# Jeremy-Cleland/hmer-img2latex

Hardware: AMD Instinct MI355X
Metric: decoded LaTeX tokens/sec at batch 256, 320x64 imgs, seq 150 (higher is better)
Workload: dtype f32

## Files before the change

### hmer-img2latex_amd/csrc/api.hip

```cpp
#include "common.h"
#include <new>

extern "C" int i2l_version(void) { return 110; }

extern "C" const char* i2l_error_string(int code) {
    switch (code) {
        case I2L_OK: return "ok";
        case I2L_ERR_ARG: return "invalid argument (null pointer or non-positive dimension)";
        case I2L_ERR_UNSUPPORTED: return "dimension not supported by the gfx950 kernels";
        case I2L_ERR_WORKSPACE: return "workspace missing or too small";
        case I2L_ERR_LAUNCH: return "HIP launch error";
        default: return "unknown error";
    }
}

struct i2l_lanes {
    int n = 0;
    hipStream_t s[I2L_MAX_LANES] = {};
    hipEvent_t fork[I2L_MAX_LANES] = {}, join[I2L_MAX_LANES] = {};
};

extern "C" int i2l_lanes_create(const i2l_stream_t* streams, int n, i2l_lanes** out) {
    if (!streams || !out || n < 1 || n > I2L_MAX_LANES) return I2L_ERR_ARG;
    for (int i = 0; i < n; ++i)
        if (!streams[i]) return I2L_ERR_ARG;
    i2l_lanes* l = new (std::nothrow) i2l_lanes();
    if (!l) return I2L_ERR_WORKSPACE;
    l->n = n;
    bool ok = true;
    for (int i = 0; i < n; ++i) {
        l->s[i] = i2l_s(streams[i]);
        ok = ok && hipEventCreateWithFlags(&l->fork[i], hipEventDisableTiming) == hipSuccess;
        ok = ok && hipEventCreateWithFlags(&l->join[i], hipEventDisableTiming) == hipSuccess;
    }
    if (!ok) { i2l_lanes_destroy(l); return I2L_ERR_LAUNCH; }
    *out = l;
// ... 48 lines not shown
```

### hmer-img2latex_amd/csrc/common.h

```cpp
#pragma once
#include <hip/hip_runtime.h>
#include <stdint.h>

#include "../../include/img2latex_hip.h"

#define I2L_CHECK_LAUNCH()                                   \
    do {                                                     \
        if (hipGetLastError() != hipSuccess) return I2L_ERR_LAUNCH; \
    } while (0)

static inline hipStream_t i2l_s(i2l_stream_t s) { return reinterpret_cast<hipStream_t>(s); }
hipStream_t i2l_side_fork(i2l_lanes* lanes, hipStream_t main, int lane);
#include <atomic>
static inline bool i2l_lds_attr(const void* fn, size_t bytes, std::atomic<unsigned>& done) {
    int dev = 0;
    if (hipGetDevice(&dev) != hipSuccess) return false;
    if (dev >= 0 && dev < 32 && ((done.load(std::memory_order_relaxed) >> dev) & 1u)) return true;
    if (hipFuncSetAttribute(fn, hipFuncAttributeMaxDynamicSharedMemorySize, (int)bytes) != hipSuccess) return false;
    if (dev >= 0 && dev < 32) done.fetch_or(1u << dev, std::memory_order_relaxed);
    return true;
}
static inline int i2l_cdiv(int a, int b) { return (a + b - 1) / b; }
static inline size_t i2l_align(size_t x, size_t a = 256) { return (x + a - 1) / a * a; }

struct GemmArgs {
    const float* A; long lda; int a_kc;
    const float* W; long ldw; int w_kc;
    long bsa, bsw; int nz;
    const float* bias;
    const float* bias2;
    float* C; int ldc;
    int M, N, K;
    int relu;
    int perm_h;
    float alpha;
    int accumulate;
    int split_bf16;
    int conv_h, conv_w;
    const float* pool_y;
    const unsigned char* pool_am;
    const float* scale;
    const float* residual;
};
static inline GemmArgs gemm_args() {
    GemmArgs g{};
    g.a_kc = 1; g.w_kc = 1; g.nz = 1; g.alpha = 1.f;
    return g;
}
size_t i2l_gemm_workspace_bytes(int M, int N, int K, int nz = 1);
int i2l_gemm(const GemmArgs& g, void* ws, size_t ws_bytes, hipStream_t s);
bool i2l_gemm_split_bf16_ok(const GemmArgs& g);

bool i2l_conv_bf16x3_applicable(int Cin, int Cout);
bool i2l_conv_bf16x3_full_applicable(int Cin, int Cout);
size_t i2l_conv_bf16x3_workspace_bytes(int Cin, int Cout);
int i2l_conv_bf16x3_run(const float* x, const float* w, const float* bias, float* y, unsigned char* amax, int B, int Cin,
                        int H, int W, int Cout, void* workspace, size_t workspace_bytes, hipStream_t s, int full = 0,
                        int weights_packed = 0);
bool i2l_conv_smallk_applicable(int Cin, int Cout);
int i2l_conv_smallk_run(const float* x, const float* w, const float* bias, float* y, unsigned char* amax, int B, int Cin,
                        int H, int W, int Cout, void* workspace, size_t workspace_bytes, hipStream_t s);
size_t i2l_conv_fixlist_bytes(void);
```

### hmer-img2latex_amd/csrc/decode.hip

```cpp
#include <math.h>
#include <stdlib.h>

#include "common.h"

namespace {

#include "lstm_rows.inc.h"

constexpr int MAXL = I2L_MAX_LSTM_LAYERS;
constexpr int NT = 256;
constexpr int VCHUNK = 2 * NT;

constexpr size_t GROUP_STATUS_BYTES = 2048;
inline bool group_shape_ok(int V, int H, int L) { return L == 1 && H == 256 && V <= 512; }

__global__ __launch_bounds__(256) void transpose_perm_kernel(const float* __restrict__ W, int N, int K,
                                                             float* __restrict__ out, int ld_out, int Npad,
                                                             int perm_h) {
    __shared__ float tile[64][65];
    const int c0 = blockIdx.x * 64, k0 = blockIdx.y * 64;
    const int tx = threadIdx.x & 63, ty = threadIdx.x >> 6;
    for (int i = ty; i < 64; i += 4) {
        const int c = c0 + i, k = k0 + tx;
        const int n = perm_h > 0 ? (c & 3) * perm_h + (c >> 2) : c;
// ... 717 lines not shown
        hipLaunchKernelGGL(transpose_perm_kernel, grid, dim3(256), 0, s, w->w_out, V, H, F(lo.WoutT), lo.Vp, lo.Vp, 0);
        I2L_CHECK_LAUNCH();
        hipLaunchKernelGGL(bout_pad_kernel, dim3(i2l_cdiv(lo.Vp, 256)), dim3(256), 0, s, w->b_out, F(lo.boutP), V, lo.Vp);
        I2L_CHECK_LAUNCH();
        if (lo.wpack16) {
            hipLaunchKernelGGL(pack16_kernel, dim3(16 * 4), dim3(64), 0, s, F(lo.WhhT[0]), F(lo.WoutT),
                               reinterpret_cast<u32x4_t*>(base + lo.wpack16));
            I2L_CHECK_LAUNCH();
        }
    }
    const size_t gws = lo.total - lo.gemm_ws;
    if (what & I2L_PREP_WEIGHTS) {
        GemmArgs g = gemm_args();
        g.A = w->embedding; g.lda = E;
        g.W = w->w_ih[0]; g.ldw = 2 * E;
        g.C = F(lo.P); g.ldc = G;
        g.M = V; g.N = G; g.K = E; g.perm_h = H;
        rc = i2l_gemm(g, base + lo.gemm_ws, gws, s);
        if (rc != I2L_OK) return rc;
    }
    if (what & I2L_PREP_ROWS) {
        GemmArgs g = gemm_args();
        g.A = enc; g.lda = E;
        g.W = w->w_ih[0] + E; g.ldw = 2 * E;
        g.bias = w->b_ih[0]; g.bias2 = w->b_hh[0];
        g.C = F(lo.Genc); g.ldc = G;
        g.M = rows; g.N = G; g.K = E; g.perm_h = H;
        rc = i2l_gemm(g, base + lo.gemm_ws, gws, s);
        if (rc != I2L_OK) return rc;
    }
    return I2L_OK;
}

namespace {
int launch_decode(const i2l_decoder_weights* w, const void* workspace, int rows, int steps, const int32_t* tok0,
                  const int32_t* forced, const float* h0, const float* c0, float temperature, int select, int stop,
                  int end_id, int top_k, float top_p, unsigned long long seed, int32_t* ids_out, float* logits_out,
                  float* probs_out, float* h_out, float* c_out, i2l_stream_t stream, int rows_per_wg = 0, int flags = 0,
                  uint32_t* resident_flag = nullptr, uint32_t resident_value = 0);
}

extern "C" int i2l_greedy_decode_ex(const i2l_decoder_weights* w, const void* workspace, int rows, int steps,
                                    const int32_t* tok0, const int32_t* forced, const float* h0, const float* c0,
                                    float temperature, int select, int stop, int end_id, int rows_per_workgroup,
                                    int32_t* ids_out, float* logits_out, float* h_out, float* c_out, int flags,
                                    uint32_t* resident_flag, uint32_t resident_value, i2l_stream_t stream) {
    if (select != I2L_SELECT_LOGITS && select != I2L_SELECT_SOFTMAX) return I2L_ERR_ARG;
    if (rows_per_workgroup != 0 && rows_per_workgroup != 1 && rows_per_workgroup != 2 && rows_per_workgroup != 4)
        return I2L_ERR_ARG;
    return launch_decode(w, workspace, rows, steps, tok0, forced, h0, c0, temperature, select, stop, end_id, 0, 0.f, 0ull,
                         ids_out, logits_out, nullptr, h_out, c_out, stream, rows_per_workgroup, flags, resident_flag,
                         resident_value);
}

extern "C" int i2l_greedy_decode(const i2l_decoder_weights* w, const void* workspace, int rows, int steps,
                                 const int32_t* tok0, const int32_t* forced, const float* h0, const float* c0,
                                 float temperature, int select, int stop, int end_id, int32_t* ids_out,
                                 float* logits_out, float* h_out, float* c_out, i2l_stream_t stream) {
    if (select != I2L_SELECT_LOGITS && select != I2L_SELECT_SOFTMAX) return I2L_ERR_ARG;
    return launch_decode(w, workspace, rows, steps, tok0, forced, h0, c0, temperature, select, stop, end_id, 0, 0.f, 0ull,
                         ids_out, logits_out, nullptr, h_out, c_out, stream);
}

extern "C" int i2l_sample_decode(const i2l_decoder_weights* w, const void* workspace, int rows, int steps,
                                 const int32_t* tok0, const float* h0, const float* c0, float temperature, int top_k,
                                 float top_p, uint64_t seed, int stop, int end_id, int32_t* ids_out, float* probs_out,
// ... 540 lines not shown
```

### hmer-img2latex_amd/csrc/gemm.hip

```cpp
#include <stdlib.h>

#include "common.h"

namespace {

#include "bf16_split.inc.h"

constexpr int BM = 64, BN = 64, BK = 64, LDP = BK + 1;
constexpr int NLD = BM * BK / 4 / 256;
constexpr int KQ = BK / 4;
typedef float f32x16 __attribute__((ext_vector_type(16)));

__host__ __device__ __forceinline__ size_t slab_stride(int M, int N) {
    size_t units = ((size_t)M * N + 63) / 64;
    if ((units & 1) == 0) ++units;
    return units * 64;
}

__device__ __forceinline__ int perm_col(int n, int perm_h) {
    if (perm_h <= 0) return n;
    const int g = n / perm_h, j = n - g * perm_h;
    return 4 * j + g;
}

// ... 428 lines not shown

int run_bf16x3(const GemmArgs& g, void* ws, size_t ws_bytes, hipStream_t s) {
    int S, kc;
    plan_bf16x3(g.M, g.N, (long)g.nz * g.K, &S, &kc);
    if (S > 1 && (!ws || ws_bytes < (size_t)S * slab_stride(g.M, g.N) * sizeof(float))) return I2L_ERR_WORKSPACE;
    const int mt = bf16x3_mt(g.M);
    const int tiles_n = i2l_cdiv(g.N, LBN), tiles = i2l_cdiv(g.M, 64 * mt) * tiles_n;
    const long long blocks = (long long)tiles * S;
    if (blocks > 0x7fffffffll) return I2L_ERR_UNSUPPORTED;
    dim3 grid((unsigned)blocks);
    float* wsf = static_cast<float*>(ws);
    const bool plain = g.nz == 1 && !g.pool_y && g.conv_h <= 0;
    if (!plain && (g.scale || g.residual)) return I2L_ERR_UNSUPPORTED;
#define I2L_LAUNCH_BF16X3(AK, WK)                                                                                          \
    do {                                                                                                                \
        if (mt == 2 && plain) hipLaunchKernelGGL((gemm_bf16x3_kernel<AK, WK, 2, true>), grid, dim3(256), 0, s, g, wsf, kc, S, tiles_n, tiles); \
        else if (mt == 2) hipLaunchKernelGGL((gemm_bf16x3_kernel<AK, WK, 2, false>), grid, dim3(256), 0, s, g, wsf, kc, S, tiles_n, tiles); \
        else if (plain) hipLaunchKernelGGL((gemm_bf16x3_kernel<AK, WK, 1, true>), grid, dim3(256), 0, s, g, wsf, kc, S, tiles_n, tiles); \
        else hipLaunchKernelGGL((gemm_bf16x3_kernel<AK, WK, 1, false>), grid, dim3(256), 0, s, g, wsf, kc, S, tiles_n, tiles);  \
    } while (0)
    if (g.a_kc && g.w_kc) I2L_LAUNCH_BF16X3(true, true);
    else if (g.a_kc) I2L_LAUNCH_BF16X3(true, false);
    else if (g.w_kc) I2L_LAUNCH_BF16X3(false, true);
    else I2L_LAUNCH_BF16X3(false, false);
#undef I2L_LAUNCH_BF16X3
    I2L_CHECK_LAUNCH();
    if (S > 1) {
        launch_splitk_reduce(g, (const float*)ws, S, s);
        I2L_CHECK_LAUNCH();
    }
    return I2L_OK;
}

}

bool i2l_gemm_split_bf16_ok(const GemmArgs& g0) {
    GemmArgs g = g0;
    if (g.nz < 1) g.nz = 1;
    return g.split_bf16 && bf16x3_applicable(g);
}

size_t i2l_gemm_workspace_bytes(int M, int N, int K, int nz) {
    int ks, kc;
    plan(M, N, K, nz < 1 ? 1 : nz, &ks, &kc);
    const size_t slabs = (size_t)ks * (nz < 1 ? 1 : nz);
    size_t need = slabs > 1 ? i2l_align(slabs * slab_stride(M, N) * sizeof(float)) : 0;
    if (K >= 64) {
        int S, kc;
        plan_bf16x3(M, N, (long)(nz < 1 ? 1 : nz) * K, &S, &kc);
        const size_t n3 = S > 1 ? i2l_align((size_t)S * slab_stride(M, N) * sizeof(float)) : 0;
        if (n3 > need) need = n3;
    }
    return need;
}

int i2l_gemm(const GemmArgs& g0, void* ws, size_t ws_bytes, hipStream_t stream) {
    GemmArgs g = g0;
    if (!g.A || !g.W || !g.C || g.M <= 0 || g.N <= 0 || g.K <= 0) return I2L_ERR_ARG;
    if (g.nz < 1) g.nz = 1;
    if (g.split_bf16 && bf16x3_applicable(g)) return run_bf16x3(g, ws, ws_bytes, stream);
    int ks, kc;
    plan(g.M, g.N, g.K, g.nz, &ks, &kc);
    const int slabs = ks * g.nz;
    if (slabs > 65535) return I2L_ERR_UNSUPPORTED;
    if (slabs > 1 && (!ws || ws_bytes < (size_t)slabs * slab_stride(g.M, g.N) * sizeof(float))) return I2L_ERR_WORKSPACE;
    auto al16 = [](const void* p) { return reinterpret_cast<uintptr_t>(p) % 16 == 0; };
// ... 123 lines not shown
```

### hmer-img2latex_amd/img2latex_amd/_lib.py

```python
from __future__ import annotations

import ctypes
import os
from ctypes import POINTER, c_char_p, c_double, c_float, c_int, c_int32, c_size_t, c_uint64, c_void_p
from typing import Optional, Sequence

import torch

_HERE = os.path.dirname(os.path.abspath(__file__))
LIB_PATH = os.path.join(_HERE, "libimg2latex_hip.so")

OK = 0
ERR_ARG, ERR_UNSUPPORTED, ERR_WORKSPACE, ERR_LAUNCH = -1, -2, -3, -4
STOP_NONE, STOP_STICKY = 0, 1
SELECT_LOGITS, SELECT_SOFTMAX, SELECT_SAMPLE = 0, 1, 2
PREP_WEIGHTS, PREP_ROWS, PREP_ALL = 1, 2, 3
MAX_LSTM_LAYERS, MAX_BEAM, MAX_NBEST = 4, 8, 16
FLAG_EXACT_FP32, FLAG_NO_GROUP, FLAG_RESNET_NO_RING, FLAG_RESNET_IM2COL_STEM = 0x1, 0x2, 0x4, 0x8
FLAG_WEIGHTS_PACKED = 0x10
FLAG_AGENT_SCOPE_EXCHANGE = 0x20
FLAG_CONV_NO_SPARSE_WGRAD = 0x4000
FLAG_CONV_COL_READY = 0x10000
FLAG_DECODE_REGION_CLEARED = 0x2000000
FLAG_RESNET_WIDE_TILES = 0x40000
# ... 32 lines not shown

_SIGNATURES = {
    "i2l_version": (c_int, []),
    "i2l_error_string": (c_char_p, [c_int]),
    "i2l_lanes_create": (c_int, [POINTER(c_void_p), c_int, POINTER(c_void_p)]),
    "i2l_lanes_destroy": (c_int, [c_void_p]),
    "i2l_lanes_join": (c_int, [c_void_p, c_void_p]),
    "i2l_stream_wait_value32": (c_int, [c_void_p, ctypes.c_uint32, ctypes.c_float, c_void_p]),
    "i2l_conv_workspace_bytes": (c_size_t, [c_int, c_int]),
    "i2l_conv3x3_relu_pool2_fwd": (c_int, [c_void_p, c_void_p, c_void_p, c_void_p, c_void_p, c_int, c_int, c_int,
                                           c_int, c_int, c_void_p, c_size_t, c_int, c_void_p]),
    "i2l_conv_bwd_workspace_bytes": (c_size_t, [c_int, c_int, c_int, c_int, c_int]),
    "i2l_conv3x3_relu_pool2_bwd": (c_int, [c_void_p, c_void_p, c_void_p, c_void_p, c_void_p, c_void_p, c_void_p,
                                           c_void_p, c_int, c_int, c_int, c_int, c_int, c_void_p, c_size_t, c_int,
                                           c_void_p, c_void_p]),
    "i2l_linear_bwd_workspace_bytes": (c_size_t, [c_int, c_int, c_int]),
    "i2l_linear_bias_act_bwd": (c_int, [c_void_p, c_void_p, c_void_p, c_void_p, c_void_p, c_void_p, c_void_p, c_int,
                                        c_int, c_int, c_int, c_void_p, c_size_t, c_int, c_void_p, c_void_p]),
    "i2l_linear_workspace_bytes": (c_size_t, [c_int, c_int, c_int]),
    "i2l_linear_bias_act_fwd": (c_int, [c_void_p, c_void_p, c_void_p, c_void_p, c_int, c_int, c_int, c_int,
                                        c_void_p, c_size_t, c_int, c_void_p]),
    "i2l_conv_bf16_packed_bytes": (c_size_t, [c_int] * 4),
    "i2l_conv_bn_bf16_pack": (c_int, [c_void_p, c_void_p, c_void_p, c_void_p, c_void_p, c_float, c_void_p, c_size_t,
                                      c_int, c_int, c_int, c_int, c_void_p]),
    "i2l_conv_bf16_workspace_bytes": (c_size_t, [c_int] * 10),
    "i2l_conv_bn_act_bf16_fwd": (c_int, [c_void_p, c_int, c_void_p, c_void_p, c_void_p] + [c_int] * 10 +
                                 [c_void_p, c_size_t, c_int, c_void_p]),
    "i2l_bottleneck_join_bf16_fwd": (c_int, [c_void_p, c_void_p, c_void_p, c_void_p, c_void_p, c_void_p, ctypes.c_long,
                                             c_int, c_int, c_int, c_void_p]),
    "i2l_maxpool3x3s2_bf16_fwd": (c_int, [c_void_p, c_void_p, c_int, c_int, c_int, c_int, c_void_p]),
    "i2l_global_avgpool_bf16_fwd": (c_int, [c_void_p, c_void_p, c_int, c_int, c_int, c_int, c_void_p]),
    "i2l_decoder_workspace_bytes": (c_size_t, [c_int, c_int, c_int, c_int, c_int]),
    "i2l_decoder_prepare": (c_int, [POINTER(DecoderWeights), c_void_p, c_int, c_int, c_void_p, c_size_t, c_void_p]),
    "i2l_greedy_decode": (c_int, [POINTER(DecoderWeights), c_void_p, c_int, c_int, c_void_p, c_void_p, c_void_p,
                                  c_void_p, c_float, c_int, c_int, c_int, c_void_p, c_void_p, c_void_p, c_void_p,
                                  c_void_p]),
    "i2l_greedy_decode_ex": (c_int, [POINTER(DecoderWeights), c_void_p, c_int, c_int, c_void_p, c_void_p, c_void_p,
                                     c_void_p, c_float, c_int, c_int, c_int, c_int, c_void_p, c_void_p, c_void_p,
                                     c_void_p, c_int, c_void_p, ctypes.c_uint32, c_void_p]),
    "i2l_greedy_decode_halves": (c_int, [POINTER(DecoderWeights), POINTER(DecodeHalf), POINTER(DecodeHalf), c_float, c_int,
                                         c_int, c_int, c_int, c_void_p, ctypes.c_uint32, c_void_p]),
    "i2l_decode_batched_scratch_bytes": (c_size_t, [c_int, c_int, c_int, c_int]),
    "i2l_greedy_decode_batched": (c_int, [POINTER(DecoderWeights), c_void_p, c_int, c_int, c_void_p, c_void_p, c_void_p,
                                          c_void_p, c_float, c_int, c_int, c_int, c_void_p, c_void_p, c_void_p, c_void_p,
                                          c_void_p, c_size_t, c_int, c_void_p, ctypes.c_uint32, c_void_p]),
    "i2l_sample_decode": (c_int, [POINTER(DecoderWeights), c_void_p, c_int, c_int, c_void_p, c_void_p, c_void_p, c_float,
                                  c_int, c_float, c_uint64, c_int, c_int, c_void_p, c_void_p, c_void_p, c_void_p,
                                  c_void_p]),
    "i2l_sample_decode_batched": (c_int, [POINTER(DecoderWeights), c_void_p, c_int, c_int, c_void_p, c_void_p, c_void_p,
                                          c_float, c_int, c_float, c_uint64, c_int, c_int, c_void_p, c_void_p, c_void_p,
                                          c_void_p, c_void_p, c_size_t, c_int, c_void_p]),
    "i2l_sample_logits": (c_int, [c_void_p, c_int, c_int, c_int, c_float, c_int, c_float, c_uint64, c_int, c_void_p,
                                  c_void_p, c_void_p]),
    "i2l_beam_workspace_bytes": (c_size_t, [c_int, c_int, c_int, c_int, c_int]),
    "i2l_beam_decode": (c_int, [POINTER(DecoderWeights), c_void_p, c_int, c_int, c_int, c_int, c_int, c_void_p,
                                c_size_t, c_void_p, c_void_p, c_void_p, c_int, c_void_p]),
    "i2l_beam_batched_scratch_bytes": (c_size_t, [c_int] * 6),
    "i2l_beam_decode_batched": (c_int, [POINTER(DecoderWeights), c_void_p, c_int, c_int, c_int, c_int, c_int, c_void_p,
                                        c_size_t, c_void_p, c_void_p, c_void_p, c_int, c_void_p]),
    "i2l_beam_nbest_scratch_bytes": (c_size_t, [c_int] * 7),
    "i2l_beam_decode_nbest": (c_int, [POINTER(DecoderWeights), c_void_p, c_int, c_int, c_int, c_int, c_int, c_int, c_void_p,
                                      c_void_p, c_size_t, c_void_p, c_void_p, c_void_p, c_void_p, c_void_p, c_void_p, c_int,
                                      c_void_p]),
    "i2l_attention_context_fwd": (c_int, [c_void_p, c_void_p, c_void_p, c_void_p, c_void_p, c_void_p, c_int, c_int,
                                          c_int, c_int, c_void_p]),
    "i2l_decoder_train_workspace_bytes": (c_size_t, [c_int, c_int, c_int, c_int, c_int, c_int]),
# ... 182 lines not shown
```

### hmer-img2latex_amd/img2latex_amd/model/lstm_decoder.py

```python
from __future__ import annotations

import ctypes
from typing import NamedTuple, Optional, Tuple

import torch
import torch.nn as nn

from .. import _lib

Hidden = Tuple[torch.Tensor, torch.Tensor]


class Attention(nn.Module):

    def __init__(self, hidden_dim: int, encoder_dim: int):
        super().__init__()
        self.hidden_dim, self.encoder_dim = hidden_dim, encoder_dim
        self.attn = nn.Linear(hidden_dim + encoder_dim, hidden_dim)
        self.v = nn.Linear(hidden_dim, 1, bias=False)

    def forward(self, hidden: torch.Tensor, encoder_outputs: torch.Tensor) -> torch.Tensor:
        hidden = _lib.require_gpu(hidden, "hidden")
        enc = _lib.require_gpu(encoder_outputs, "encoder_outputs")
        B, S, E = enc.shape
# ... 60 lines not shown
        w.w_out, w.b_out = wout.data_ptr(), bout.data_ptr()
        w.vocab, w.embed, w.hidden, w.layers = self.vocab_size, self.embedding_dim, self.hidden_dim, L
        return w, (tens, emb, wout, bout, arrs)

    def _weights_version(self):
        return tuple((p.data_ptr(), p._version) for p in self.parameters())

    def prepare(self, encoder_output: torch.Tensor, reuse_weight_images: bool = True, slot=None):
        enc = _lib.require_gpu(encoder_output, "encoder_output")
        if enc.dim() != 2 or enc.shape[1] != self.embedding_dim:
            raise RuntimeError(f"encoder_output must be (B,{self.embedding_dim}), got {tuple(enc.shape)}")
        rows = enc.shape[0]
        L = _lib.lib()
        w, keep = self._weights_struct()
        nbytes = L.i2l_decoder_workspace_bytes(rows, self.vocab_size, self.embedding_dim, self.hidden_dim,
                                               self.lstm_layers)
        if nbytes == 0:
            raise RuntimeError("img2latex_amd: decoder dimensions not supported by the HIP kernels")
        key = (rows, enc.device, self._weights_version())
        what = _lib.PREP_ALL
        sid = _lib.stream_ptr() if slot is None else ("slot", slot)
        self._ws, self._ws_key = self._ws_by_stream.get(sid, (None, None))
        if self._ws is None or self._ws.numel() < nbytes or self._ws.device != enc.device:
            self._ws = torch.empty(nbytes, dtype=torch.uint8, device=enc.device)
            self._ws_key = None
        if reuse_weight_images and self._ws_key == key:
            what = _lib.PREP_ROWS
        _lib.check(L.i2l_decoder_prepare(ctypes.byref(w), enc.data_ptr(), rows, what, self._ws.data_ptr(),
                                         self._ws.numel(), _lib.stream_ptr()), "decoder_prepare")
        self._ws_key = key
        self._ws_by_stream[sid] = (self._ws, key)
        _lib.mark("prepare")
        return w, keep, enc

    def release_slots(self, owner) -> None:
        for sid in [k for k in self._ws_by_stream
                    if isinstance(k, tuple) and k[0] == "slot" and isinstance(k[1], tuple) and len(k[1]) > 1 and k[1][1] == owner]:
            ws, _ = self._ws_by_stream.pop(sid)
            if self._ws is ws:
                self._ws, self._ws_key = None, None

    def group_status(self):
        if self._ws is None or self._ws_key is None:
            return None
        off = _lib.lib().i2l_decoder_group_status_offset(self._ws_key[0], self.vocab_size, self.embedding_dim,
                                                         self.hidden_dim, self.lstm_layers)
        if off == 0:
            return None
        st = self._ws[off:off + 16].view(torch.int32).cpu().tolist()
        return {"timed_out": bool(st[0]), "groups": st[1], "groups_on_one_xcd": st[2]}

    def run_steps(self, encoder_output: torch.Tensor, steps: int, tok0: torch.Tensor,
                  forced: Optional[torch.Tensor] = None, hidden: Optional[Hidden] = None,
                  temperature: float = 1.0, select: int = _lib.SELECT_LOGITS, stop: int = _lib.STOP_NONE,
                  end_id: int = -1, want_ids: bool = True, want_logits: bool = False,
                  want_state: bool = False, reuse_weight_images: bool = True, rows_per_workgroup: int = 0,
                  flags: int = 0, prepared=None, resident=None):
        if prepared is None:
            w, keep, enc = self.prepare(encoder_output, reuse_weight_images)
            ws = self._ws
        else:
            w, keep, enc, ws = prepared
        rows, dev = enc.shape[0], enc.device
        tok0 = _lib.require_gpu(tok0, "tok0", torch.int32)
        if forced is not None:
            forced = _lib.require_gpu(forced, "forced", torch.int32)
# ... 155 lines not shown
```

### hmer-img2latex_amd/img2latex_amd/pipeline.py

```python
from __future__ import annotations

from collections import deque
from typing import Deque, List, Optional, Tuple

import torch

from . import _lib
from .model.lstm_decoder import DecodeHalf


class _Batch:
    __slots__ = ("no", "done", "host", "enc", "text", "half", "slot", "ids")

    def __init__(self, no, host, enc, slot):
        self.no, self.host, self.enc, self.slot = no, host, enc, slot
        self.done = self.text = self.half = self.ids = None


class GreedyPipeline:

    def __init__(self, model, start_token_id: int, end_token_id: int, max_length: int = 150,
                 temperature: float = 1.0, depth: int = 3, rows_per_workgroup: int = 2, decode_streams: int = 1,
                 decode_flags: int = 0, encoder_flags: int = 0, decode_priority: int = 0, encoder_streams: int = 1,
                 encoder_priority: int = 0, hold_encoder: Optional[bool] = None, wait_timeout_us: float = 20000.0,
                 clear_early: bool = True,
                 stop: int = _lib.STOP_NONE, select: int = _lib.SELECT_LOGITS, detokenize=None,
                 split_decode: Optional[bool] = None):
        self.model = model
        self.start, self.end, self.max_length, self.temperature = start_token_id, end_token_id, max_length, temperature
        dev = next(model.parameters()).device
        if dev.type != "cuda":
            raise RuntimeError("img2latex_amd: GreedyPipeline needs the model on a ROCm device (no CPU fallback)")
        self.device = dev
        self.enc_streams = [torch.cuda.Stream(device=dev, priority=int(encoder_priority)) for _ in range(max(1, encoder_streams))]
        self._next_enc = 0
        self.dec_streams = [torch.cuda.Stream(device=dev, priority=int(decode_priority)) for _ in range(max(1, decode_streams))]
        self._next_dec = 0
        self.depth = max(depth, len(self.dec_streams) + len(self.enc_streams))
        self.rows_per_workgroup = rows_per_workgroup
        self.decode_flags = int(decode_flags)
        self.stop, self.select = int(stop), int(select)
        self.encoder_flags = int(encoder_flags)
        if len(self.enc_streams) >= 2:
            self.encoder_flags |= getattr(model.encoder, "MULTI_STREAM_FLAGS", 0)
        if hold_encoder is None:
            hold_encoder = bool(self.decode_flags & (_lib.FLAG_DECODE_GROUP8 | _lib.FLAG_DECODE_GROUP16))
        self.hold_encoder = bool(hold_encoder)
        self.clear_early = bool(clear_early)
        self.wait_timeout_us = float(wait_timeout_us)
        self._resident = torch.zeros(1, dtype=torch.int32, device=dev)
        self.trace: Optional[list] = None
        self.trace_every = 1
        self._inflight: Deque[_Batch] = deque()
        dec = model.decoder
        can_split = (bool(self.decode_flags & _lib.FLAG_DECODE_GROUP16) and self.stop == _lib.STOP_NONE
                     and len(self.dec_streams) == 1 and self.rows_per_workgroup == 0 and max_length >= 8
                     and not (int(getattr(dec, "kernel_flags", 0)) & _lib.FLAG_DECODE_BATCHED)
                     and hasattr(dec, "halves_supported") and dec.halves_supported(self.stop))
        if split_decode and not can_split:
            raise RuntimeError("img2latex_amd: GreedyPipeline(split_decode=True) needs decode_flags with FLAG_DECODE_GROUP16, "
                               "rows_per_workgroup=0, stop=STOP_NONE, one decode stream, max_length >= 8 and a decoder the "
                               "16-member grouped kernel takes")
        self.split_decode = can_split if split_decode is None else bool(split_decode)
        self._open: Optional[_Batch] = None
        self._tok0: dict = {}
        self.copy_stream = torch.cuda.Stream(device=dev)
        self._batch_no = 0
        self._slots = self.depth + 1
        self._free: List[torch.Tensor] = []
        self._lent: Optional[torch.Tensor] = None
        self.detok = detokenize
        self._text_dev: dict = {}
        self._text_free: List[Tuple[torch.Tensor, torch.Tensor]] = []

    def submit(self, images: torch.Tensor) -> None:
        if len(self._inflight) >= self.depth:
            raise RuntimeError(f"GreedyPipeline: {self.depth} batches already in flight; collect() first")
        cur = torch.cuda.current_stream(self.device)
        enc_stream = self.enc_streams[self._next_enc]
        self._next_enc = (self._next_enc + 1) % len(self.enc_streams)
        enc_stream.wait_stream(cur)
        with torch.no_grad():
            with torch.cuda.stream(enc_stream):
                if self.hold_encoder and self._batch_no >= len(self.enc_streams):
                    _lib.check(_lib.lib().i2l_stream_wait_value32(
                        self._resident.data_ptr(), self._batch_no - len(self.enc_streams) + 1, self.wait_timeout_us,
                        _lib.stream_ptr()), "stream_wait_value32")
                rec = None
                if self.trace is not None and self._batch_no % self.trace_every < 2:
                    rec = {k: torch.cuda.Event(enable_timing=True) for k in ("enc_start", "enc_end", "dec_start", "dec_end")}
                    rec["batch"] = self._batch_no
                    rec["enc_start"].record(enc_stream)
                    self.trace.append(rec)
                saved = self.model.encoder.kernel_flags
                self.model.encoder.kernel_flags = saved | self.encoder_flags
                try:
                    enc = self.model.encoder(images)
                finally:
                    self.model.encoder.kernel_flags = saved
                slot = self._batch_no % self._slots
                seq = self._batch_no + 1
                self._batch_no += 1
                dec = self.model.decoder
                w, keep, enc_c = dec.prepare(enc, slot=("pipe", id(self), slot))
                prepared = (w, keep, enc_c, dec._ws)
                dflags = self.decode_flags
                if self.clear_early and dflags & (_lib.FLAG_DECODE_GROUP8 | _lib.FLAG_DECODE_GROUP16):
                    dims = (enc.shape[0], dec.vocab_size, dec.embedding_dim, dec.hidden_dim, dec.lstm_layers)
                    off = _lib.lib().i2l_decoder_group_status_offset(*dims)
                    nb = _lib.lib().i2l_decoder_group_region_bytes(*dims)
                    if off and nb:
                        dec._ws[off:off + nb].zero_()
                        dflags |= _lib.FLAG_DECODE_REGION_CLEARED
                enc_done = torch.cuda.Event() if rec is None else rec["enc_end"]
                enc_done.record(enc_stream)
            images.record_stream(enc_stream)
            dec_stream = self.dec_streams[self._next_dec]
            self._next_dec = (self._next_dec + 1) % len(self.dec_streams)
            with torch.cuda.stream(dec_stream):
                dec_stream.wait_event(enc_done)
                enc.record_stream(dec_stream)
                if rec is not None:
                    rec["dec_start"].record(dec_stream)
                if self.split_decode:
                    self._submit_split(enc, prepared, slot, seq, dflags, rec, dec_stream)
                    return
                ids, _ = self.model.greedy_ids(enc, self.start, self.end, self.max_length, self.temperature,
                                               stop=self.stop, select=self.select,
                                               rows_per_workgroup=self.rows_per_workgroup, flags=dflags,
                                               prepared=prepared,
                                               resident=(self._resident, seq) if self.hold_encoder else None)
                if rec is not None:
                    rec["dec_end"].record(dec_stream)
                b = _Batch(seq - 1, self._host_buffer(ids.shape), enc, slot)
                b.ids = ids
                self._finish(b, dec_stream)
        self._inflight.append(b)

    def _finish(self, b: _Batch, dec_stream) -> None:
        ids, host, slot = b.ids, b.host, b.slot
        text = dev_text = None
        if self.detok is not None:
            key = (slot, tuple(ids.shape))
            if key not in self._text_dev:
                self._text_dev = {k: v for k, v in self._text_dev.items() if k[0] != slot}
                self._text_dev[key] = self.detok.buffers(*ids.shape)
            dev_text = self.detok.launch(ids, self.end, self._text_dev[key])
            text = self._text_buffer(dev_text)
        if self.copy_stream is None:
            host.copy_(ids, non_blocking=True)
            if text is not None:
                text[0].copy_(dev_text[0], non_blocking=True)
                text[1].copy_(dev_text[1], non_blocking=True)
            done = torch.cuda.Event()
            done.record(dec_stream)
        else:
            decoded = torch.cuda.Event()
            decoded.record(dec_stream)
            self.copy_stream.wait_event(decoded)
            with torch.cuda.stream(self.copy_stream):
                host.copy_(ids, non_blocking=True)
                if text is not None:
                    text[0].copy_(dev_text[0], non_blocking=True)
                    text[1].copy_(dev_text[1], non_blocking=True)
                done = torch.cuda.Event()
                done.record(self.copy_stream)
            ids.record_stream(self.copy_stream)
        b.text, b.done, b.half, b.ids = text, done, None, None

    def _submit_split(self, enc, prepared, slot, seq, dflags, rec, dec_stream) -> None:
# ... 134 lines not shown
```

### include/img2latex_hip.h

```cpp
#ifndef IMG2LATEX_HIP_H
#define IMG2LATEX_HIP_H

#include <stddef.h>
#include <stdint.h>

#ifdef __cplusplus
extern "C" {
#endif

#define I2L_OK 0
#define I2L_ERR_ARG (-1)
#define I2L_ERR_UNSUPPORTED (-2)
#define I2L_ERR_WORKSPACE (-3)
#define I2L_ERR_LAUNCH (-4)

#define I2L_MAX_LSTM_LAYERS 4
#define I2L_MAX_BEAM 8
#define I2L_MAX_NBEST 16

typedef void* i2l_stream_t;

#define I2L_FLAG_EXACT_FP32 0x1
#define I2L_FLAG_NO_GROUP 0x2
#define I2L_FLAG_RESNET_NO_RING 0x4
// ... 82 lines not shown
int i2l_conv_bn_act_f32_fwd(const float* x, int x_kind, const float* w, const float* scale, const float* shift,
                            const float* residual, float* y, int B, int H, int W, int Cin, int Cout, int kh, int kw,
                            int stride, int pad, int relu, void* workspace, size_t workspace_bytes, int flags,
                            i2l_stream_t stream);
int i2l_im2col_f32(const void* x, int x_kind, int B, int H, int W, int C, int kh, int kw, int stride, int pad,
                   float* col, i2l_stream_t stream);
int i2l_col2im_f32(const float* dcol, int B, int H, int W, int C, int kh, int kw, int stride, int pad, float* dx,
                   int accumulate, i2l_stream_t stream);
int i2l_maxpool3x3s2_f32_fwd(const float* x, float* y, int B, int H, int W, int C, i2l_stream_t stream);
int i2l_maxpool3x3s2_f32_bwd(const float* x, const float* dy, float* dx, int B, int H, int W, int C, i2l_stream_t stream);
int i2l_global_avgpool_f32_fwd(const float* x, float* y, int B, int H, int W, int C, i2l_stream_t stream);
int i2l_global_avgpool_bwd_f32(const float* dfeat, float* dx, int B, int H, int W, int C, i2l_stream_t stream);


typedef struct i2l_decoder_weights {
    const float* embedding;
    const float* const* w_ih;
    const float* const* w_hh;
    const float* const* b_ih;
    const float* const* b_hh;
    const float* w_out;
    const float* b_out;
    int vocab, embed, hidden, layers;
} i2l_decoder_weights;

size_t i2l_decoder_workspace_bytes(int rows, int vocab, int embed, int hidden, int layers);

#define I2L_PREP_WEIGHTS 1
#define I2L_PREP_ROWS 2
#define I2L_PREP_ALL 3
int i2l_decoder_prepare(const i2l_decoder_weights* w, const float* enc, int rows, int what,
                        void* workspace, size_t workspace_bytes, i2l_stream_t stream);

#define I2L_STOP_NONE 0
#define I2L_STOP_STICKY 1

#define I2L_SELECT_LOGITS 0
#define I2L_SELECT_SOFTMAX 1
#define I2L_SELECT_SAMPLE 2

int i2l_greedy_decode(const i2l_decoder_weights* w, const void* workspace, int rows, int steps,
                      const int32_t* tok0, const int32_t* forced, const float* h0, const float* c0,
                      float temperature, int select, int stop, int end_id,
                      int32_t* ids_out, float* logits_out, float* h_out, float* c_out,
                      i2l_stream_t stream);

int i2l_greedy_decode_ex(const i2l_decoder_weights* w, const void* workspace, int rows, int steps,
                         const int32_t* tok0, const int32_t* forced, const float* h0, const float* c0,
                         float temperature, int select, int stop, int end_id, int rows_per_workgroup,
                         int32_t* ids_out, float* logits_out, float* h_out, float* c_out, int flags,
                         uint32_t* resident_flag, uint32_t resident_value, i2l_stream_t stream);

size_t i2l_decode_batched_scratch_bytes(int rows, int vocab, int hidden, int layers);
int i2l_greedy_decode_batched(const i2l_decoder_weights* w, const void* workspace, int rows, int steps,
                              const int32_t* tok0, const int32_t* forced, const float* h0, const float* c0,
                              float temperature, int select, int stop, int end_id, int32_t* ids_out,
                              float* logits_out, float* h_out, float* c_out, void* scratch, size_t scratch_bytes,
                              int flags, uint32_t* resident_flag, uint32_t resident_value, i2l_stream_t stream);

int i2l_sample_decode(const i2l_decoder_weights* w, const void* workspace, int rows, int steps,
                      const int32_t* tok0, const float* h0, const float* c0, float temperature, int top_k,
                      float top_p, uint64_t seed, int stop, int end_id, int32_t* ids_out, float* probs_out,
                      float* h_out, float* c_out, i2l_stream_t stream);

int i2l_sample_decode_batched(const i2l_decoder_weights* w, const void* workspace, int rows, int steps,
                              const int32_t* tok0, const float* h0, const float* c0, float temperature, int top_k,
// ... 214 lines not shown
```

Measured before the change: 41.14 million.

## Fuse encoder FC tail with decoder prep and region clear in pipeline

Result: no change. 41.30 million, median of 3 (+0.4%).

```diff
diff --git a/hmer-img2latex_amd/csrc/api.hip b/hmer-img2latex_amd/csrc/api.hip
--- a/hmer-img2latex_amd/csrc/api.hip
+++ b/hmer-img2latex_amd/csrc/api.hip
@@ -1,7 +1,7 @@
 #include "common.h"
 #include <new>
 
-extern "C" int i2l_version(void) { return 110; }
+extern "C" int i2l_version(void) { return 111; }
 
 extern "C" const char* i2l_error_string(int code) {
     switch (code) {
diff --git a/hmer-img2latex_amd/csrc/common.h b/hmer-img2latex_amd/csrc/common.h
--- a/hmer-img2latex_amd/csrc/common.h
+++ b/hmer-img2latex_amd/csrc/common.h
@@ -50,6 +50,7 @@
 size_t i2l_gemm_workspace_bytes(int M, int N, int K, int nz = 1);
 int i2l_gemm(const GemmArgs& g, void* ws, size_t ws_bytes, hipStream_t s);
 bool i2l_gemm_split_bf16_ok(const GemmArgs& g);
+int i2l_encoder_tail_fc(const GemmArgs& g, void* ws, size_t ws_bytes, void* clear, size_t clear_bytes, hipStream_t s);
 
 bool i2l_conv_bf16x3_applicable(int Cin, int Cout);
 bool i2l_conv_bf16x3_full_applicable(int Cin, int Cout);
diff --git a/hmer-img2latex_amd/csrc/decode.hip b/hmer-img2latex_amd/csrc/decode.hip
--- a/hmer-img2latex_amd/csrc/decode.hip
+++ b/hmer-img2latex_amd/csrc/decode.hip
@@ -773,6 +773,34 @@
     return I2L_OK;
 }
 
+extern "C" int i2l_encoder_tail_fwd(const float* features, const float* fc_weight, const float* fc_bias, float* enc_out,
+                                    const i2l_decoder_weights* w, int rows, int K, void* decoder_workspace,
+                                    size_t decoder_workspace_bytes, void* fc_workspace, size_t fc_workspace_bytes,
+                                    int flags, i2l_stream_t stream) {
+    if (!features || !fc_weight || !enc_out || rows <= 0 || K <= 0) return I2L_ERR_ARG;
+    int rc = check_weights(w);
+    if (rc != I2L_OK) return rc;
+    if (flags & ~I2L_FLAG_EXACT_FP32) return I2L_ERR_ARG;
+    if ((flags & I2L_FLAG_EXACT_FP32) || K < 2048 || K % 8 != 0) return I2L_ERR_UNSUPPORTED;
+    const int V = w->vocab, E = w->embed, H = w->hidden, L = w->layers;
+    const Layout lo = make_layout(rows, V, E, H, L);
+    if (!decoder_workspace || decoder_workspace_bytes < lo.total) return I2L_ERR_WORKSPACE;
+    if (!fc_workspace || fc_workspace_bytes < i2l_linear_workspace_bytes(rows, K, E)) return I2L_ERR_WORKSPACE;
+    char* base = static_cast<char*>(decoder_workspace);
+    hipStream_t s = i2l_s(stream);
+    GemmArgs g = gemm_args();
+    g.A = features; g.lda = K;
+    g.W = fc_weight; g.ldw = K;
+    g.bias = fc_bias;
+    g.C = enc_out; g.ldc = E;
+    g.M = rows; g.N = E; g.K = K;
+    g.relu = 1;
+    g.split_bf16 = 1;
+    rc = i2l_encoder_tail_fc(g, fc_workspace, fc_workspace_bytes, base + lo.xchg, lo.xchg ? lo.xchg_bytes : 0, s);
+    if (rc != I2L_OK) return rc;
+    return i2l_decoder_prepare(w, enc_out, rows, I2L_PREP_ROWS, decoder_workspace, decoder_workspace_bytes, stream);
+}
+
 namespace {
 int launch_decode(const i2l_decoder_weights* w, const void* workspace, int rows, int steps, const int32_t* tok0,
                   const int32_t* forced, const float* h0, const float* c0, float temperature, int select, int stop,
diff --git a/hmer-img2latex_amd/csrc/encoder_tail.inc.h b/hmer-img2latex_amd/csrc/encoder_tail.inc.h
--- /dev/null
+++ b/hmer-img2latex_amd/csrc/encoder_tail.inc.h
@@ -0,0 +1,159 @@
+
+constexpr int TBM = 128, TBN = 128, TLP = 128 + 2;
+constexpr int TIMG = 3 * 4 * TLP;
+constexpr int TAIL_LDS_BYTES = 2 * 2 * TIMG * 16;
+
+__global__ __launch_bounds__(256, 2) void fc_tail_bf16x3_kernel(GemmArgs g, float* __restrict__ partial, int k_chunk,
+                                                                int S, int tiles_n, int tiles) {
+    extern __shared__ __attribute__((aligned(16))) uint4 tail_lds[];
+    auto image = [&](int buf, int operand) { return tail_lds + ((buf & 1) * 2 + operand) * TIMG; };
+    const int tid = threadIdx.x, lane = tid & 63, wave = tid >> 6;
+    const int wm = wave >> 1, wn = wave & 1;
+    const int i = lane & 31, h = lane >> 5;
+    const int L = blockIdx.x;
+    int tile, slice;
+    if ((S & 7) == 0) { const int grp = L >> 3; tile = grp % tiles; slice = (L & 7) + 8 * (grp / tiles); }
+    else { tile = L % tiles; slice = L / tiles; }
+    if (slice >= S) return;
+    const int m0 = (tile / tiles_n) * TBM, n0 = (tile % tiles_n) * TBN;
+    const int kbeg = slice * k_chunk, kend = min(g.K, kbeg + k_chunk);
+
+    const int row = tid >> 2, kg = tid & 3;
+    bool oka[2], okw[2];
+    unsigned oa[2], ow[2];
+#pragma unroll
+    for (int p = 0; p < 2; ++p) {
+        oka[p] = m0 + row + 64 * p < g.M;
+        okw[p] = n0 + row + 64 * p < g.N;
+        oa[p] = (unsigned)min(m0 + row + 64 * p, g.M - 1) * (unsigned)g.lda * 4u;
+        ow[p] = (unsigned)min(n0 + row + 64 * p, g.N - 1) * (unsigned)g.ldw * 4u;
+    }
+    const char* const abase = reinterpret_cast<const char*>(g.A);
+    const char* const wbase = reinterpret_cast<const char*>(g.W);
+    struct Stage { float4 a[2][2], w[2][2]; };
+    auto fetch = [&](Stage& st, int k0) {
+        const int k = k0 + kg * 8;
+        const unsigned kb = (unsigned)min(k, kend - 8) * 4u;
+#pragma unroll
+        for (int p = 0; p < 2; ++p) {
+            const float4 alo = *reinterpret_cast<const float4*>(abase + (oa[p] + kb)), ahi = *reinterpret_cast<const float4*>(abase + (oa[p] + kb + 16u));
+            const float4 wlo = *reinterpret_cast<const float4*>(wbase + (ow[p] + kb)), whi = *reinterpret_cast<const float4*>(wbase + (ow[p] + kb + 16u));
+            st.a[p][0] = alo; st.a[p][1] = ahi;
+            st.w[p][0] = wlo; st.w[p][1] = whi;
+        }
+    };
+    auto split_part = [&](const Stage& st, int k0, uint4* a_s, uint4* w_s, int q, unsigned (&pc)[3][4]) {
+        const int p = q >> 3, operand = (q >> 2) & 1, pr = q & 3;
+        const float4& lo = operand ? st.w[p][0] : st.a[p][0];
+        const float4& hi = operand ? st.w[p][1] : st.a[p][1];
+        const bool in = k0 + kg * 8 < kend && (operand ? okw[p] : oka[p]);
+        const float x = in ? (pr == 0 ? lo.x : pr == 1 ? lo.z : pr == 2 ? hi.x : hi.z) : 0.f;
+        const float y = in ? (pr == 0 ? lo.y : pr == 1 ? lo.w : pr == 2 ? hi.y : hi.w) : 0.f;
+        split3_pair(x, y, pc[0][pr], pc[1][pr], pc[2][pr]);
+        if (pr == 3) {
+            uint4* dst = operand ? w_s : a_s;
+#pragma unroll
+            for (int sp = 0; sp < 3; ++sp)
+                dst[(sp * 4 + kg) * TLP + row + 64 * p] = make_uint4(pc[sp][0], pc[sp][1], pc[sp][2], pc[sp][3]);
+        }
+    };
+    auto commit = [&](const Stage& st, int k0, uint4* a_s, uint4* w_s) {
+        unsigned pc[3][4];
+#pragma unroll
+        for (int q = 0; q < 16; ++q) split_part(st, k0, a_s, w_s, q, pc);
+    };
+
+    f32x16 acc[2][2];
+#pragma unroll
+    for (int m = 0; m < 2; ++m)
+#pragma unroll
+        for (int n = 0; n < 2; ++n)
+#pragma unroll
+            for (int r = 0; r < 16; ++r) acc[m][n][r] = 0.f;
+
+    auto step = [&](Stage& nxt, int j, int k0) {
+        const uint4* a_s = image(j, 0);
+        const uint4* w_s = image(j, 1);
+        uint4* a_n = image(j + 1, 0);
+        uint4* w_n = image(j + 1, 1);
+        unsigned pc[3][4];
+#pragma unroll
+        for (int s = 0; s < 2; ++s) {
+            i16x8_t a[2][3];
+#pragma unroll
+            for (int sp = 0; sp < 3; ++sp)
+#pragma unroll
+                for (int m = 0; m < 2; ++m) {
+                    const uint4 t = a_s[(sp * 4 + s * 2 + h) * TLP + wm * 64 + m * 32 + i];
+                    a[m][sp] = *reinterpret_cast<const i16x8_t*>(&t);
+                }
+#pragma unroll
+            for (int n = 0; n < 2; ++n) {
+                i16x8_t b[3];
+#pragma unroll
+                for (int sp = 0; sp < 3; ++sp) {
+                    const uint4 t = w_s[(sp * 4 + s * 2 + h) * TLP + wn * 64 + n * 32 + i];
+                    b[sp] = *reinterpret_cast<const i16x8_t*>(&t);
+                }
+                constexpr int TI[6] = {0, 1, 2, 0, 1, 0}, TJ[6] = {2, 1, 0, 1, 0, 0};
+#pragma unroll
+                for (int t = 0; t < 6; ++t)
+#pragma unroll
+                    for (int m = 0; m < 2; ++m) {
+                        acc[m][n] = __builtin_amdgcn_mfma_f32_32x32x16_bf16(a[m][TI[t]], b[TJ[t]], acc[m][n], 0, 0, 0);
+                        const int u = ((s * 2 + n) * 6 + t) * 2 + m;
+                        if (u % 3 == 0) split_part(nxt, k0 + LBK, a_n, w_n, u / 3, pc);
+                    }
+            }
+        }
+        fetch(nxt, k0 + 3 * LBK);
+        __syncthreads();
+    };
+    Stage st0, st1;
+    fetch(st0, kbeg);
+    fetch(st1, kbeg + LBK);
+    commit(st0, kbeg, image(0, 0), image(0, 1));
+    fetch(st0, kbeg + 2 * LBK);
+    __syncthreads();
+    for (int j = 0, k0 = kbeg; k0 < kend; j += 2, k0 += 2 * LBK) {
+        step(st1, j, k0);
+        if (k0 + LBK >= kend) break;
+        step(st0, j + 1, k0 + LBK);
+    }
+    float* slab = partial + (size_t)slice * slab_stride(g.M, g.N);
+#pragma unroll
+    for (int m = 0; m < 2; ++m)
+#pragma unroll
+        for (int n = 0; n < 2; ++n) {
+            const int col = n0 + wn * 64 + n * 32 + i;
+#pragma unroll
+            for (int r = 0; r < 16; ++r) {
+                const int rw = m0 + wm * 64 + m * 32 + (r & 3) + 8 * (r >> 2) + 4 * h;
+                if (rw < g.M && col < g.N) slab[(size_t)rw * g.N + col] = acc[m][n][r];
+            }
+        }
+}
+
+__global__ __launch_bounds__(256) void encoder_tail_finish_kernel(GemmArgs g, const float* __restrict__ partial, int slabs,
+                                                                  unsigned* __restrict__ clear, size_t clear_words) {
+    const size_t total = (size_t)g.M * g.N, stride = slab_stride(g.M, g.N);
+    const size_t t0 = (size_t)blockIdx.x * 256 + threadIdx.x, nt = (size_t)gridDim.x * 256;
+    for (size_t e = t0; e < total; e += nt) {
+        const int m = (int)(e / g.N), n = (int)(e - (size_t)m * g.N);
+        float v = 0.f;
+        int s = 0;
+        for (; s + 32 <= slabs; s += 32) {
+            float t[32];
+#pragma unroll
+            for (int j = 0; j < 32; ++j) t[j] = partial[(size_t)(s + j) * stride + e];
+#pragma unroll
+            for (int j = 0; j < 32; ++j) v += t[j];
+        }
+        for (; s < slabs; ++s) v += partial[(size_t)s * stride + e];
+        epilogue_store(g, m, n, v);
+    }
+    uint4* c4 = reinterpret_cast<uint4*>(clear);
+    const size_t n4 = clear_words / 4;
+    for (size_t e = t0; e < n4; e += nt) c4[e] = make_uint4(0u, 0u, 0u, 0u);
+    for (size_t e = n4 * 4 + t0; e < clear_words; e += nt) clear[e] = 0u;
+}
diff --git a/hmer-img2latex_amd/csrc/gemm.hip b/hmer-img2latex_amd/csrc/gemm.hip
--- a/hmer-img2latex_amd/csrc/gemm.hip
+++ b/hmer-img2latex_amd/csrc/gemm.hip
@@ -484,6 +484,36 @@
     return I2L_OK;
 }
 
+#include "encoder_tail.inc.h"
+
+}
+
+int i2l_encoder_tail_fc(const GemmArgs& g, void* ws, size_t ws_bytes, void* clear, size_t clear_bytes, hipStream_t s) {
+    auto al16 = [](const void* p) { return reinterpret_cast<uintptr_t>(p) % 16 == 0; };
+    if (!g.split_bf16 || g.nz != 1 || !g.a_kc || !g.w_kc || g.pool_y || g.conv_h > 0 || !bf16x3_applicable(g))
+        return I2L_ERR_UNSUPPORTED;
+    if (clear_bytes % 4 != 0 || !al16(clear)) return I2L_ERR_UNSUPPORTED;
+    if ((unsigned long long)g.M * g.lda >= (1ull << 30) || (unsigned long long)g.N * g.ldw >= (1ull << 30))
+        return I2L_ERR_UNSUPPORTED;
+    int S, kc;
+    plan_bf16x3(g.M, g.N, g.K, &S, &kc);
+    if (!ws || ws_bytes < (size_t)S * slab_stride(g.M, g.N) * sizeof(float)) return I2L_ERR_WORKSPACE;
+    const int tiles_n = i2l_cdiv(g.N, TBN), tiles = i2l_cdiv(g.M, TBM) * tiles_n;
+    const long long blocks = (long long)tiles * S;
+    if (blocks > 0x7fffffffll) return I2L_ERR_UNSUPPORTED;
+    float* wsf = static_cast<float*>(ws);
+    if (hipFuncSetAttribute(reinterpret_cast<const void*>(fc_tail_bf16x3_kernel), hipFuncAttributeMaxDynamicSharedMemorySize,
+                            TAIL_LDS_BYTES) != hipSuccess)
+        return I2L_ERR_LAUNCH;
+    hipLaunchKernelGGL(fc_tail_bf16x3_kernel, dim3((unsigned)blocks), dim3(256), TAIL_LDS_BYTES, s, g, wsf, kc, S, tiles_n, tiles);
+    I2L_CHECK_LAUNCH();
+    const size_t total = (size_t)g.M * g.N;
+    int rb = (int)((total + 255) / 256);
+    if (rb > 2048) rb = 2048;
+    hipLaunchKernelGGL(encoder_tail_finish_kernel, dim3(rb), dim3(256), 0, s, g, (const float*)wsf, S,
+                       static_cast<unsigned*>(clear), clear_bytes / 4);
+    I2L_CHECK_LAUNCH();
+    return I2L_OK;
 }
 
 bool i2l_gemm_split_bf16_ok(const GemmArgs& g0) {
diff --git a/hmer-img2latex_amd/img2latex_amd/_lib.py b/hmer-img2latex_amd/img2latex_amd/_lib.py
--- a/hmer-img2latex_amd/img2latex_amd/_lib.py
+++ b/hmer-img2latex_amd/img2latex_amd/_lib.py
@@ -88,6 +88,8 @@
     "i2l_global_avgpool_bf16_fwd": (c_int, [c_void_p, c_void_p, c_int, c_int, c_int, c_int, c_void_p]),
     "i2l_decoder_workspace_bytes": (c_size_t, [c_int, c_int, c_int, c_int, c_int]),
     "i2l_decoder_prepare": (c_int, [POINTER(DecoderWeights), c_void_p, c_int, c_int, c_void_p, c_size_t, c_void_p]),
+    "i2l_encoder_tail_fwd": (c_int, [c_void_p, c_void_p, c_void_p, c_void_p, POINTER(DecoderWeights), c_int, c_int,
+                                     c_void_p, c_size_t, c_void_p, c_size_t, c_int, c_void_p]),
     "i2l_greedy_decode": (c_int, [POINTER(DecoderWeights), c_void_p, c_int, c_int, c_void_p, c_void_p, c_void_p,
                                   c_void_p, c_float, c_int, c_int, c_int, c_void_p, c_void_p, c_void_p, c_void_p,
                                   c_void_p]),
diff --git a/hmer-img2latex_amd/img2latex_amd/model/lstm_decoder.py b/hmer-img2latex_amd/img2latex_amd/model/lstm_decoder.py
--- a/hmer-img2latex_amd/img2latex_amd/model/lstm_decoder.py
+++ b/hmer-img2latex_amd/img2latex_amd/model/lstm_decoder.py
@@ -116,6 +116,17 @@
         self._ws_by_stream[sid] = (self._ws, key)
         _lib.mark("prepare")
         return w, keep, enc
+
+    def slot_prepared(self, slot) -> bool:
+        return self._ws_by_stream.get(("slot", slot), (None, None))[1] is not None
+
+    def claim_prepared(self, rows: int, device, slot):
+        sid = ("slot", slot)
+        ws, key = self._ws_by_stream.get(sid, (None, None))
+        if ws is None or key is None or key != (rows, device, self._weights_version()):
+            return None
+        self._ws, self._ws_key = ws, key
+        return self._weights_struct()
 
     def release_slots(self, owner) -> None:
         for sid in [k for k in self._ws_by_stream
diff --git a/hmer-img2latex_amd/img2latex_amd/pipeline.py b/hmer-img2latex_amd/img2latex_amd/pipeline.py
--- a/hmer-img2latex_amd/img2latex_amd/pipeline.py
+++ b/hmer-img2latex_amd/img2latex_amd/pipeline.py
@@ -1,5 +1,6 @@
 from __future__ import annotations
 
+import ctypes
 from collections import deque
 from typing import Deque, List, Optional, Tuple
 
@@ -25,7 +26,7 @@
                  encoder_priority: int = 0, hold_encoder: Optional[bool] = None, wait_timeout_us: float = 20000.0,
                  clear_early: bool = True,
                  stop: int = _lib.STOP_NONE, select: int = _lib.SELECT_LOGITS, detokenize=None,
-                 split_decode: Optional[bool] = None):
+                 split_decode: Optional[bool] = None, tail_fused: Optional[bool] = None):
         self.model = model
         self.start, self.end, self.max_length, self.temperature = start_token_id, end_token_id, max_length, temperature
         dev = next(model.parameters()).device
@@ -62,6 +63,11 @@
                                "rows_per_workgroup=0, stop=STOP_NONE, one decode stream, max_length >= 8 and a decoder the "
                                "16-member grouped kernel takes")
         self.split_decode = can_split if split_decode is None else bool(split_decode)
+        from .model.cnn_encoder import CNNEncoder
+        can_fuse = isinstance(model.encoder, CNNEncoder) and hasattr(dec, "claim_prepared")
+        if tail_fused and not can_fuse:
+            raise RuntimeError("img2latex_amd: GreedyPipeline(tail_fused=True) needs a CNNEncoder and an LSTMDecoder")
+        self.tail_fused = can_fuse if tail_fused is None else bool(tail_fused)
         self._open: Optional[_Batch] = None
         self._tok0: dict = {}
         self.copy_stream = torch.cuda.Stream(device=dev)
@@ -95,17 +101,25 @@
                 saved = self.model.encoder.kernel_flags
                 self.model.encoder.kernel_flags = saved | self.encoder_flags
                 try:
-                    enc = self.model.encoder(images)
+                    fused = self._encoder_tail(images) if self.tail_fused else None
+                    enc = self.model.encoder(images) if fused is None else fused[0]
+                    if fused is not None and fused[1] is None:
+                        fused = None
                 finally:
                     self.model.encoder.kernel_flags = saved
                 slot = self._batch_no % self._slots
                 seq = self._batch_no + 1
                 self._batch_no += 1
                 dec = self.model.decoder
-                w, keep, enc_c = dec.prepare(enc, slot=("pipe", id(self), slot))
+                if fused is None:
+                    w, keep, enc_c = dec.prepare(enc, slot=("pipe", id(self), slot))
+                else:
+                    w, keep, enc_c = fused[1], fused[2], enc
                 prepared = (w, keep, enc_c, dec._ws)
                 dflags = self.decode_flags
-                if self.clear_early and dflags & (_lib.FLAG_DECODE_GROUP8 | _lib.FLAG_DECODE_GROUP16):
+                if fused is not None:
+                    dflags |= _lib.FLAG_DECODE_REGION_CLEARED
+                elif self.clear_early and dflags & (_lib.FLAG_DECODE_GROUP8 | _lib.FLAG_DECODE_GROUP16):
                     dims = (enc.shape[0], dec.vocab_size, dec.embedding_dim, dec.hidden_dim, dec.lstm_layers)
                     off = _lib.lib().i2l_decoder_group_status_offset(*dims)
                     nb = _lib.lib().i2l_decoder_group_region_bytes(*dims)
@@ -136,6 +150,42 @@
                 b.ids = ids
                 self._finish(b, dec_stream)
         self._inflight.append(b)
+
+    def _encoder_tail(self, images: torch.Tensor):
+        encoder, dec = self.model.encoder, self.model.decoder
+        if (encoder.kernel_flags & _lib.FLAG_EXACT_FP32) or not (self.clear_early and self.decode_flags & _lib.FLAG_DECODE_GROUP16):
+            return None
+        if images.dim() != 4:
+            return None
+        rows, K, E = images.shape[0], encoder.flattened_size, encoder.embedding_dim
+        L = _lib.lib()
+        dims = (rows, dec.vocab_size, dec.embedding_dim, dec.hidden_dim, dec.lstm_layers)
+        if (E != dec.embedding_dim or K < 2048 or K % 8 or not L.i2l_decoder_group_status_offset(*dims)
+                or not L.i2l_decoder_group_region_bytes(*dims)):
+            return None
+        if not dec.slot_prepared(("pipe", id(self), self._batch_no % self._slots)):
+            return None
+        feat = encoder.conv_blocks(images)[-1]
+        if feat.numel() != rows * K:
+            raise RuntimeError(f"flattened size {feat.numel() // rows} != embedding_layer.in_features {K} "
+                               "(image size differs from the constructor's)")
+        claimed = dec.claim_prepared(rows, images.device, ("pipe", id(self), self._batch_no % self._slots))
+        if claimed is None:
+            return encoder._linear(feat), None, None
+        w, keep = claimed
+        enc = torch.empty((rows, E), dtype=torch.float32, device=feat.device)
+        nbytes = L.i2l_linear_workspace_bytes(rows, K, E)
+        ws = encoder._workspace(nbytes, feat.device)
+        wt = _lib.require_gpu(encoder.embedding_layer.weight.detach(), "embedding_layer.weight")
+        bs = _lib.require_gpu(encoder.embedding_layer.bias.detach(), "embedding_layer.bias")
+        rc = L.i2l_encoder_tail_fwd(feat.data_ptr(), wt.data_ptr(), bs.data_ptr(), enc.data_ptr(), ctypes.byref(w), rows, K,
+                                    dec._ws.data_ptr(), dec._ws.numel(), _lib.ptr(ws), nbytes, 0, _lib.stream_ptr())
+        if rc == _lib.ERR_UNSUPPORTED:
+            return encoder._linear(feat), None, None
+        _lib.check(rc, "encoder_tail_fwd")
+        _lib.mark("fc")
+        _lib.mark("prepare")
+        return enc, w, keep
 
     def _finish(self, b: _Batch, dec_stream) -> None:
         ids, host, slot = b.ids, b.host, b.slot
diff --git a/include/img2latex_hip.h b/include/img2latex_hip.h
--- a/include/img2latex_hip.h
+++ b/include/img2latex_hip.h
@@ -138,6 +138,11 @@
 int i2l_decoder_prepare(const i2l_decoder_weights* w, const float* enc, int rows, int what,
                         void* workspace, size_t workspace_bytes, i2l_stream_t stream);
 
+int i2l_encoder_tail_fwd(const float* features, const float* fc_weight, const float* fc_bias, float* enc_out,
+                         const i2l_decoder_weights* w, int rows, int K, void* decoder_workspace,
+                         size_t decoder_workspace_bytes, void* fc_workspace, size_t fc_workspace_bytes, int flags,
+                         i2l_stream_t stream);
+
 #define I2L_STOP_NONE 0
 #define I2L_STOP_STICKY 1
 
diff --git a/profiles/encoder_tail_cost.py b/profiles/encoder_tail_cost.py
--- /dev/null
+++ b/profiles/encoder_tail_cost.py
@@ -0,0 +1,72 @@
+import argparse
+import csv
+import statistics
+
+
+def short(name):
+    return name.replace("(anonymous namespace)::", "").replace("void ", "").split("(")[0].strip()[:56]
+
+
+def main():
+    ap = argparse.ArgumentParser()
+    ap.add_argument("trace")
+    ap.add_argument("--steps", type=int, default=100)
+    ap.add_argument("--out", default=None)
+    a = ap.parse_args()
+    rows = [r for r in csv.DictReader(open(a.trace))]
+    for r in rows:
+        r["t0"], r["t1"] = int(r["Start_Timestamp"]), int(r["End_Timestamp"])
+    rows.sort(key=lambda r: r["t0"])
+    two_tile = [r for r in rows if "decode_group16_kernel<2" in r["Kernel_Name"]]
+    if not two_tile:
+        raise SystemExit("no decode_group16_kernel<2> launch in the trace: not a pipelined bench.py run")
+    region_end = two_tile[-1]["t1"]
+    qkey = "Queue_Id" if "Queue_Id" in rows[0] else "Stream_Id"
+    chains = {}
+    for r in rows:
+        if r["t0"] < region_end:
+            chains.setdefault(r[qkey], []).append(r)
+    enc_q = max(chains, key=lambda q: sum("conv3x3_smallk" in r["Kernel_Name"] for r in chains[q]))
+    seq = chains[enc_q]
+    batches, i = [], 0
+    while i < len(seq):
+        if "conv3x3" in seq[i]["Kernel_Name"] and i + 1 < len(seq) and "conv3x3" not in seq[i + 1]["Kernel_Name"]:
+            j = i + 1
+            while j < len(seq) and "conv3x3" not in seq[j]["Kernel_Name"]:
+                j += 1
+            tail = [r for r in seq[i + 1:j] if "wait" not in r["Kernel_Name"]]
+            if tail and j < len(seq):
+                batches.append((seq[i], tail))
+            i = j
+        else:
+            i += 1
+    batches = batches[-a.steps:]
+    shape = [short(r["Kernel_Name"]) for r in batches[-1][1]]
+    batches = [b for b in batches if [short(r["Kernel_Name"]) for r in b[1]] == shape]
+    out = [f"{len(batches)} batches of the timed pipelined region (encoder queue {enc_q}); us per batch: mean / median / min / max"]
+    st = lambda v: f"{statistics.mean(v):7.1f} / {statistics.median(v):7.1f} / {min(v):7.1f} / {max(v):7.1f}"
+    tot_k, tot_g = [0.0] * len(batches), [0.0] * len(batches)
+    for k, name in enumerate(shape):
+        dur = [(b[1][k]["t1"] - b[1][k]["t0"]) / 1e3 for b in batches]
+        gap = [(b[1][k]["t0"] - (b[1][k - 1]["t1"] if k else b[0]["t1"])) / 1e3 for b in batches]
+        grid = batches[-1][1][k]
+        out.append(f"  {name:56s} grid {grid['Grid_Size_X']:>7s} x {grid['Grid_Size_Y']:>4s} x {grid['Grid_Size_Z']:>3s}")
+        out.append(f"      gap in front  {st(gap)}")
+        out.append(f"      duration      {st(dur)}")
+        tot_k = [x + y for x, y in zip(tot_k, dur)]
+        tot_g = [x + y for x, y in zip(tot_g, gap)]
+    span = [(b[1][-1]["t1"] - b[0]["t1"]) / 1e3 for b in batches]
+    conv3 = [(b[0]["t1"] - b[0]["t0"]) / 1e3 for b in batches]
+    out.append(f"  tail kernels, summed                  {st(tot_k)}")
+    out.append(f"  gaps, summed                          {st(tot_g)}")
+    out.append(f"  third conv block's end -> enc_end     {st(span)}")
+    out.append(f"  (the third conv block itself          {st(conv3)})")
+    text = "\n".join(out)
+    print(text)
+    if a.out:
+        with open(a.out, "w") as f:
+            f.write(text + "\n")
+
+
+if __name__ == "__main__":
+    main()
```
